# mozilla/mozjpeg

Measured on NVIDIA H100. Metric: megapixels/sec encode (4K RGB q75 4:2:0), higher is better.
Workload: dtype u8 in / int32 DCT / fp32 trellis costs / u8 out

## Files before the change

### mozjpeg_b200/csrc/encoder.cu

```cuda
#include "b200jpeg.h"
#include "internal.h"
#include "kernels.cuh"
#include <cmath>
#include <cstdio>
#include <cstdlib>
#include <cstring>
#include <map>
#include <string>
#include <vector>

namespace b200 {

#define CU(call) do { cudaError_t e_ = (call); if (e_ != cudaSuccess) { set_error("%s failed: %s (%s:%d)", #call, cudaGetErrorString(e_), __FILE__, __LINE__); return B200JPEG_ERR_CUDA; } } while (0)

static const int kZigzag[64] = {
   0,  1,  8, 16,  9,  2,  3, 10, 17, 24, 32, 25, 18, 11,  4,  5,
  12, 19, 26, 33, 40, 48, 41, 34, 27, 20, 13,  6,  7, 14, 21, 28,
  35, 42, 49, 56, 57, 50, 43, 36, 29, 22, 15, 23, 30, 37, 44, 51,
  58, 59, 52, 45, 38, 31, 39, 46, 53, 60, 61, 54, 47, 55, 62, 63};

struct DevBuf {
  void *p = nullptr; size_t cap = 0;
  int reserve(size_t n) {
    if (n <= cap) return B200JPEG_OK;
// ... 611 lines not shown
      }
    }
    auto round = [&](const Geom &gr, const RecLayout &rlr, int bSs, int bSe) -> int {
    if (!pl.progressive) {
      if (fwd_stats) {
        tm.mark("trellis_dc_stats");
        launch_gather_comp_dc(gr, pl.rs, so.dcq, rlr, A.d_hist.as<uint32_t>(), status, n, s);
      } else {
        tm.mark("trellis_stats");
        CU(cudaMemsetAsync(A.d_hist.p, 0, hist_bytes * gr.nc, s));
        launch_gather_comp(gr, pl.rs, A.d_hist.as<uint32_t>(), status, n, s);
      }
      tm.mark("trellis_tables");
      SlotMasks masks; memset(&masks, 0, sizeof masks); masks.period = gr.nc;
      for (int ci = 0; ci < gr.nc; ci++) masks.m[ci] = (1u << gr.c[ci].dc_tbl) | (1u << (4 + gr.c[ci].ac_tbl));
      launch_gen_tables(A.d_hist.as<uint32_t>(), tset, tabset, masks, n * gr.nc, s);
    } else {
      for (int ci = 0; ci < gr.nc; ci++) {
        ScanDesc ts; memset(&ts, 0, sizeof ts);
        ts.ncomps = 1; ts.ci[0] = ci; ts.Ss = bSs; ts.Se = bSe; ts.bim = 1; ts.k_count[0] = 1;
        ts.per_row = gr.c[ci].wib; ts.rows = gr.c[ci].hib; ts.nblocks = (long long)ts.per_row * ts.rows;
        ts.ri = p->restart_in_rows > 0 ? (int)std::min((long long)p->restart_in_rows * ts.per_row, 65535LL) : p->restart_interval;
        tm.mark("trellis_stats");
        CU(cudaMemsetAsync(A.d_hist.p, 0, hist_bytes, s));
        launch_seed_hist(A.d_hist.as<uint32_t>(), 4 + gr.c[ci].ac_tbl, n, s);
        launch_prog_prepare(gr, ts, A.d_blk_aux.as<uint32_t>(), A.d_blk_run.as<uint32_t>(), A.d_blk_mask.as<unsigned long long>(), A.d_tile_bits.as<int>(), A.d_tile_base.as<int>(), n, s);
        launch_gather_prog(gr, ts, A.d_blk_aux.as<uint32_t>(), A.d_blk_run.as<uint32_t>(), A.d_blk_mask.as<unsigned long long>(), A.d_hist.as<uint32_t>(), status, n, s);
        tm.mark("trellis_tables");
        SlotMasks masks; memset(&masks, 0, sizeof masks); masks.period = 1; masks.m[0] = 1u << (4 + gr.c[ci].ac_tbl);
        launch_gen_tables(A.d_hist.as<uint32_t>(), tset + (size_t)ci * HIST_SLOTS, tabset * gr.nc, masks, n, s);
      }
    }
    if (!generic_rounds) {
      tm.mark("trellis_ac");
      if (so.hist) CU(cudaMemsetAsync(A.d_hist.p, 0, hist_bytes, s));
      launch_trellis_ac3(gr, e->d_tc.as<TrellisConsts>(), tset, tabset, A.d_rec.as<DcRec>(), rlr, A.d_srec.p, A.d_splits.as<uint32_t>(), so, n, e->sms, s);
    } else {
      tm.mark("trellis_ac");
      float4 *eo = eobopt ? A.d_eo.as<float4>() : nullptr;
      launch_trellis_ac_band(gr, e->d_tc.as<TrellisConsts>(), tset, tabset, A.d_rec.as<DcRec>(), rlr, bSs, bSe, qimg, eo, n, s);
      if (eobopt) launch_trellis_eob_rows(gr, tset, tabset, A.d_rec.as<DcRec>(), rlr, bSs, bSe, eo, A.d_es.p, n, s);
      if (qopt) launch_qopt_sums(gr, A.d_qsum.as<long long>(), n, s);
    }
    if (p->trellis_quant_dc) {
      tm.mark("trellis_dc");
      if (pl.progressive) launch_trellis_dc(gr, e->d_tc.as<TrellisConsts>(), e->d_tabs_fixed.as<DevHuff>(), 0, A.d_rec.as<DcRec>(), A.d_bt.as<unsigned long long>(), rlr, p->trellis_delta_dc_weight > 0.0f, dc_fast_of(gr), nullptr, 1, n, s);
      else launch_trellis_dc(gr, e->d_tc.as<TrellisConsts>(), tset, tabset, A.d_rec.as<DcRec>(), A.d_bt.as<unsigned long long>(), rlr, p->trellis_delta_dc_weight > 0.0f, dc_fast_of(gr), so.dcq, so.keep_coef, n, s);
    }
    return B200JPEG_OK;
    };
    auto band_Ss = [&](int band) { return (nband == 2 && band == 1) ? p->trellis_freq_split + 1 : 1; };
    auto band_Se = [&](int band) { return (nband == 2 && band == 0) ? p->trellis_freq_split : 63; };
    if (!qopt) {
      for (int loop = 0; loop < p->trellis_num_loops; loop++)
        for (int band = 0; band < nband; band++) { int rc = round(g, rl, band_Ss(band), band_Se(band)); if (rc) return rc; }
    } else {
      const int group = g.nc * (nband == 2 ? 4 : 2);
      int pass_number = 0;
      CU(cudaMemsetAsync(A.d_qsum.p, 0, (size_t)n * 4 * 2 * 64 * 8, s));
      for (int ci = 0; ci < g.nc; ci++) {
        Geom gs = g; gs.nc = 1; gs.c[0] = g.c[ci];
        RecLayout rls = rl; rls.comp_off[0] = rl.comp_off[ci];
        for (int loop = 0; loop < p->trellis_num_loops; loop++)
          for (int band = 0; band < nband; band++) {
            pass_number++;
            if (pass_number % group == 1) CU(cudaMemsetAsync(A.d_qsum.p, 0, (size_t)n * 4 * 2 * 64 * 8, s));
            int rc = round(gs, rls, band_Ss(band), band_Se(band)); if (rc) return rc;
            if ((pass_number + 1) % group == 0) launch_qopt_update(A.d_qsum.as<long long>(), qimg, n, s);
            pass_number++;
          }
      }
      CU(cudaMemcpyAsync(io.qimg, qimg, (size_t)n * 512, cudaMemcpyDeviceToDevice, s));
    }
    if (!fwd_stats) {
      tm.mark("dummy");
      launch_dummy(g, n, s);
    }
  }

  int *best_al = A.d_best_al.as<int>();
// ... 971 lines not shown
```

### mozjpeg_b200/csrc/kernels.cu

```cuda
#include "kernels.cuh"
#include <cuda_fp16.h>
#include <cuda.h>
#include <cstdio>
#include <cstdlib>
#include <type_traits>

namespace b200 {

unsigned long long g_kernel_launches = 0;
#define LAUNCHED() (++g_kernel_launches)

__constant__ uint8_t c_zz[64] = {
   0,  1,  8, 16,  9,  2,  3, 10, 17, 24, 32, 25, 18, 11,  4,  5,
  12, 19, 26, 33, 40, 48, 41, 34, 27, 20, 13,  6,  7, 14, 21, 28,
  35, 42, 49, 56, 57, 50, 43, 36, 29, 22, 15, 23, 30, 37, 44, 51,
  58, 59, 52, 45, 38, 31, 39, 46, 53, 60, 61, 54, 47, 55, 62, 63};
__constant__ uint8_t c_izz[64] = {
   0,  1,  5,  6, 14, 15, 27, 28,  2,  4,  7, 13, 16, 26, 29, 42,
   3,  8, 12, 17, 25, 30, 41, 43,  9, 11, 18, 24, 31, 40, 44, 53,
  10, 19, 23, 32, 39, 45, 52, 54, 20, 22, 33, 38, 46, 51, 55, 60,
  21, 34, 37, 47, 50, 56, 59, 61, 35, 36, 48, 49, 57, 58, 62, 63};
__constant__ unsigned long long c_izz_col[8] = {0x2315140a09030200ull, 0x242216130b080401ull, 0x30252117120c0705ull, 0x312f262018110d06ull, 0x39322e271f19100eull, 0x3a38332d281e1a0full, 0x3e3b37342c291d1bull, 0x3f3d3c36352b2a1cull};
#ifndef FWD_KZ_PACKED
#define FWD_KZ_PACKED 1
// ... 1922 lines not shown
      splits[4 * blockIdx.y] = start[63 - 32]; splits[4 * blockIdx.y + 1] = start[63 - mid_max]; splits[4 * blockIdx.y + 2] = start[63 - 8];
      splits[4 * blockIdx.y + 3] = (uint32_t)nblk;
    }
  }
  __syncthreads();
  if (threadIdx.x < 64) { const unsigned mine = cnt[threadIdx.x]; start[threadIdx.x] += mine ? atomicAdd(&gcur[(size_t)blockIdx.y * 64 + threadIdx.x], mine) : 0u; }
  __syncthreads();
  for (long long b = b0 + threadIdx.x; b < b1; b += blockDim.x) {
    const uint4 q = reinterpret_cast<const uint4 *>(r)[b];
    const int nz = (int)((q.y >> 16) & 0xFF);
    const unsigned pos = atomicAdd(&start[63 - min(nz, 63)], 1u);
    reinterpret_cast<uint4 *>(p)[pos] = make_uint4(q.x, (unsigned)b, q.z, q.w);
  }
}
static void launch_sort2(const Geom &g, const DcRec *rec, const RecLayout &rl, SRec *srec, uint32_t *splits, unsigned *scratch , int mid_max, int n, cudaStream_t s)
{
  long long mb = 0;
  for (int ci = 0; ci < g.nc; ci++) mb = max(mb, (long long)g.c[ci].wib * g.c[ci].hib);
  const size_t words = (size_t)n * g.nc * 64;
  cudaMemsetAsync(scratch, 0, 2 * words * sizeof(unsigned), s);
  dim3 grid((unsigned)((mb + SORT_SLICE - 1) / SORT_SLICE), n * g.nc);
  k_sort_count<<<grid, 256, 0, s>>>(g, rec, rl, scratch); LAUNCHED();
  k_sort_scatter<<<grid, 256, 0, s>>>(g, rec, rl, srec, splits, scratch, scratch + words, mid_max); LAUNCHED();
}

__device__ __forceinline__ float u2f_exact(unsigned v) { return __uint_as_float(0x4B000000u | v) - 8388608.0f; }

#define T3_THREADS 128
#ifndef SYMREC_DIRECT
#define SYMREC_DIRECT 0
#endif
static_assert(!(SYMREC_DIRECT && SYMREC_SPLIT), "the direct-store A/B aid writes whole 128-byte slots");
#ifndef T3_MINB_8
#define T3_MINB_8 8
#endif
#ifndef T3_MINB_15
#define T3_MINB_15 8
#endif
#ifndef T3_PRED_UNROLL
#define T3_PRED_UNROLL 4
#endif
#define T3_PRAGMA_(x) _Pragma(#x)
#define T3_PRAGMA_UNROLL(n) T3_PRAGMA_(unroll n)
template <int MM> struct T3Smem {
  uint2 rec[MM][T3_THREADS];
  unsigned ew[MM][T3_THREADS];
};

template <int KN>
__device__ __forceinline__ void t3_pred_loop(const int t, const uint2 *__restrict__ rec , const unsigned *__restrict__ ew ,
                                             const char *__restrict__ rb, const float before, const float d0, const float d1, const float d2,
                                             float &kb0, int &ks0, float &kb1, int &ks1, float &kb2, int &ks2)
{
T3_PRAGMA_UNROLL(T3_PRED_UNROLL)
  for (int s = 0; s < t; s++) {
    const uint2 r = rec[s * T3_THREADS];
    const int pos4 = (int)(ew[s * T3_THREADS] & 0xFCu);
    const float T = (before + __uint_as_float(r.x)) + __uint_as_float(r.y);
    const char *ra = rb - pos4;
    { const float c = (*reinterpret_cast<const float *>(ra) + d0) + T; if (c < kb0) { kb0 = c; ks0 = s + 1; } }
    if (KN > 1) { const float c = (*reinterpret_cast<const float *>(ra + 256) + d1) + T; if (c < kb1) { kb1 = c; ks1 = s + 1; } }
    if (KN > 2) { const float c = (*reinterpret_cast<const float *>(ra + 512) + d2) + T; if (c < kb2) { kb2 = c; ks2 = s + 1; } }
  }
}
__device__ __forceinline__ float t3_dist(const int cand, const int q, const int x, const float lambda, const float wl)
{
  const float fd = u2f_exact((unsigned)abs(cand * q - x));
  return ((fd * fd) * lambda) * wl;
}

// ... 47 lines not shown
  const size_t rbase = (size_t)img * rl.per_image + rl.comp_off[ci];
  const int use_norm = tc->use_norm;
  const double p1 = tc->p1, p2 = tc->p2; const float lambda_const = tc->lambda_const;
  uint2 *myrec = &L.rec[0][tid]; unsigned *myew = &L.ew[0][tid];
  const char *srate_b = reinterpret_cast<const char *>(srate);
  const float INF = __int_as_float(0x7F800000);

#pragma unroll 1
  for (int chunk = blockIdx.x; chunk < nchunks; chunk += gridDim.x) {
    const long long tix = lo + (long long)chunk * T3_THREADS + tid;
    const bool live = tix < hi;
    SRec sr; sr.norm = 0.f; sr.lin = 0; sr.nzmask = 0;
    if (live) sr = srec[rbase + tix];
    const unsigned lin = sr.lin;
    const int by = lin / c.wib, bx = lin - by * c.wib;
    const size_t blk = ((size_t)img * c.hpad + by) * c.wpad + bx;
    const int16_t *raw16 = c.raw + blk * 64;
    int16_t *o16 = c.coef + blk * 64;
    uint4 rv[8];
#pragma unroll
    for (int v = 0; v < 8; v++) rv[v] = make_uint4(0, 0, 0, 0);
    unsigned dc_q = 0;
    const bool want_dc = !so.sym || so.keep_coef || so.dcq_ac;
    if (live) {
      const uint4 *r4 = reinterpret_cast<const uint4 *>(raw16);
#pragma unroll
      for (int v = 0; v < 8; v++) rv[v] = r4[v];
      if (want_dc) dc_q = (unsigned)(unsigned short)o16[0];
    }
    float lambda;
    {
      const float norm = (float)((double)sr.norm / 63.0);
      if (use_norm) lambda = (float)(p1 / (p2 + (double)norm)); else lambda = lambda_const;
      if (live) rec[rbase + lin].lambda_dc = lambda * swz[0];
    }
    const unsigned mlo = (unsigned)sr.nzmask, mhi = (unsigned)(sr.nzmask >> 32);
    const int m = __popc(mlo) + __popc(mhi);
    const int mmax = __reduce_max_sync(0xffffffffu, m);
    float azd = 0.0f;
    if (mmax != 0) {
      uint2 *push = myrec;
      const float bias = -8421376.0f;
#pragma unroll
      for (int v = 0; v < 8; v++) {
        const unsigned aw[4] = {rv[v].x, rv[v].y, rv[v].z, rv[v].w};
        const float4 w0 = reinterpret_cast<const float4 *>(swz)[2 * v], w1 = reinterpret_cast<const float4 *>(swz)[2 * v + 1];
        const float ww[8] = {w0.x, w0.y, w0.z, w0.w, w1.x, w1.y, w1.z, w1.w};
        const unsigned mw = v < 4 ? mlo : mhi;
#pragma unroll
        for (int jj = 0; jj < 4; jj++) {
          const unsigned u = aw[jj] ^ 0x80008000u;
          const float fx = __fadd_rn(__uint_as_float(__byte_perm(u, 0x4B000000u, 0x7610)), bias);
          const float fy = __fadd_rn(__uint_as_float(__byte_perm(u, 0x4B000000u, 0x7632)), bias);
          const float2 z = make_float2(__fmul_rn(__fmul_rn(__fmul_rn(fx, fx), lambda), ww[2 * jj]),
                                       __fmul_rn(__fmul_rn(__fmul_rn(fy, fy), lambda), ww[2 * jj + 1]));
          const int i = 8 * v + 2 * jj;
          if (i != 0) {
            if (mw & (1u << (i & 31))) { *push = make_uint2(__float_as_uint(azd), __byte_perm(aw[jj], (unsigned)i, 0x1054)); push += T3_THREADS; }
            azd = z.x + azd;
          }
          if (mw & (1u << ((i + 1) & 31))) { *push = make_uint2(__float_as_uint(azd), __byte_perm(aw[jj], (unsigned)(i + 1), 0x3254)); push += T3_THREADS; }
          azd = z.y + azd;
        }
      }
    }
    const float azd63 = azd;
    int last = 0;
// ... 115 lines not shown
#else
        uint4 *dlo = reinterpret_cast<uint4 *>(so.sym + (rbase + lin) * SYMREC_BYTES), *dhi = dlo;
#endif
        for (int v = 0; 4 * v < nw; v += 2) {
          const uint2 a = myrec[(2 * v) * T3_THREADS], b = myrec[(2 * v + 1) * T3_THREADS];
          const uint2 c2 = myrec[(2 * v + 2) * T3_THREADS], d2 = myrec[(2 * v + 3) * T3_THREADS];
          uint4 *dst = v < 4 ? dlo : dhi;
          dst[v] = make_uint4(a.x, a.y, b.x, b.y);
          dst[v + 1] = make_uint4(c2.x, c2.y, d2.x, d2.y);
        }
#endif
        if (so.dcq_ac) so.dcq[rbase + lin] = (int16_t)dc_q;
        if (so.keep_coef || ns > SYMREC_SLOTS) write_block(last0);
      }
    }
  }
  if (so.hist) {
    __syncthreads();
    uint32_t *gh = so.hist + ((size_t)img * HIST_SLOTS + 4 + c.ac_tbl) * HIST_BINS;
    for (int i = tid; i < 162; i += T3_THREADS) {
      const unsigned v = shist[i];
      if (v) atomicAdd(&gh[i < 160 ? (((i / 10) << 4) | (i % 10 + 1)) : i == 160 ? 0 : 0xF0], v);
    }
  }
}

template <int MM>
static void launch_t3(dim3 grid, cudaStream_t s, const Geom &g, const TrellisConsts *tc, const DevHuff *tabs, size_t tabs_set_stride,
                      DcRec *rec, const RecLayout &rl, const SRec *srec, const uint32_t *splits, const SymOut &so)
{
  if (sizeof(T3Smem<MM>) + 8192 > 48 * 1024) cudaFuncSetAttribute(k_trellis_ac3<MM>, cudaFuncAttributeMaxDynamicSharedMemorySize, (int)sizeof(T3Smem<MM>));
  k_trellis_ac3<MM><<<grid, T3_THREADS, sizeof(T3Smem<MM>), s>>>(g, tc, tabs, tabs_set_stride, rec, rl, srec, splits, so); LAUNCHED();
}
void launch_trellis_ac3(const Geom &g, const TrellisConsts *tc, const DevHuff *tabs, size_t tabs_set_stride,
                        DcRec *rec, const RecLayout &rl, void *srec, uint32_t *splits, const SymOut &so, int n, int sms, cudaStream_t s)
{
  launch_sort2(g, rec, rl, static_cast<SRec *>(srec), splits, splits + (size_t)n * g.nc * 4, 15, n, s);
  long long mb = 0;
  for (int ci = 0; ci < g.nc; ci++) mb = max(mb, (long long)g.c[ci].wib * g.c[ci].hib);
  const unsigned full = (unsigned)((mb + T3_THREADS - 1) / T3_THREADS);
  unsigned gx = (unsigned)max(1, min((int)full, (sms * 8 * 3 + n * g.nc - 1) / (n * g.nc)));
  dim3 grid(gx, n * g.nc);
  const SRec *sr = static_cast<const SRec *>(srec);
  launch_t3<64>(dim3(min(gx, 8u), grid.y), s, g, tc, tabs, tabs_set_stride, rec, rl, sr, splits, so);
  launch_t3<32>(dim3(min(gx, 16u), grid.y), s, g, tc, tabs, tabs_set_stride, rec, rl, sr, splits, so);
  launch_t3<15>(grid, s, g, tc, tabs, tabs_set_stride, rec, rl, sr, splits, so);
  launch_t3<8>(grid, s, g, tc, tabs, tabs_set_stride, rec, rl, sr, splits, so);
}

__global__ void __launch_bounds__(256) k_dc_collect(Geom g, RecLayout rl, int16_t *__restrict__ dcq)
{
  const int ci = blockIdx.y % g.nc, img = blockIdx.y / g.nc;
  const CompGeom &c = g.c[ci];
  const long long nblk = (long long)c.wib * c.hib, t = (long long)blockIdx.x * blockDim.x + threadIdx.x;
  if (t >= nblk) return;
  const int row = (int)(t / c.wib), col = (int)(t - (long long)row * c.wib);
  dcq[(size_t)img * rl.per_image + rl.comp_off[ci] + t] = c.coef[(((size_t)img * c.hpad + row) * c.wpad + col) * 64];
}
static void launch_dc_collect(const Geom &g, const RecLayout &rl, int16_t *dcq, int n, cudaStream_t s)
{
  long long mb = 0;
  for (int ci = 0; ci < g.nc; ci++) mb = max(mb, (long long)g.c[ci].wib * g.c[ci].hib);
  dim3 grid((unsigned)((mb + 255) / 256), n * g.nc);
  k_dc_collect<<<grid, 256, 0, s>>>(g, rl, dcq); LAUNCHED();
}

__global__ void __launch_bounds__(64) k_trellis_dc(Geom g, const TrellisConsts *__restrict__ tc,
                                                   const DevHuff *__restrict__ tabs, size_t tabs_set_stride,
                                                   const DcRec *__restrict__ rec, unsigned long long *__restrict__ bt, RecLayout rl)
{
  const int ci = blockIdx.y % g.nc, img = blockIdx.y / g.nc;
  const CompGeom &c = g.c[ci];
  __shared__ uint8_t dcsi[32];
  {
    const DevHuff *dc = reinterpret_cast<const DevHuff *>(reinterpret_cast<const char *>(tabs) + (size_t)blockIdx.y * tabs_set_stride) + c.dc_tbl;
    if (threadIdx.x < 32) dcsi[threadIdx.x] = dc->size[threadIdx.x];
  }
  __syncthreads();
  int imcu = blockIdx.x * blockDim.x + threadIdx.x;
  int n_imcu = (c.hib + c.v - 1) / c.v;
  if (imcu >= n_imcu) return;
  const int q = qset_of(tc, g, img)->q8_zz[c.qt][0];
  int ncand = (2 + 60 / (q >> 3)) | 1; if (ncand > 9) ncand = 9;
  const int half = ncand / 2;
  const int lim = 1 << tc->max_coef_bits;
  int last_dc = 0;
  for (int br = 0; br < c.v; br++) {
    int row = imcu * c.v + br;
    if (row >= c.hib) break;
    size_t rbase = (size_t)img * rl.per_image + rl.comp_off[ci] + (size_t)row * c.wib;
    float acc[9]; int prevc[9];
#pragma unroll
    for (int k = 0; k < 9; k++) { acc[k] = 0.f; prevc[k] = 0; }
    for (int bi = 0; bi < c.wib; bi++) {
      DcRec r = rec[rbase + bi];
      int raw = r.raw_dc, sign = raw >> 31, x = abs(raw);
      int qval = (x + q / 2) / q;
      const bool vert = br > 0 && tc->delta_dc_weight > 0.0f;
      int above_raw = 0, above_fin = 0;
      if (vert) { above_raw = rec[rbase - c.wib + bi].raw_dc; above_fin = c.coef[(((size_t)img * c.hpad + row - 1) * c.wpad + bi) * 64]; }
      float nacc[9]; int cand[9];
      unsigned long long w = 0;
#pragma unroll
      for (int k = 0; k < 9; k++) {
        nacc[k] = 0.f; cand[k] = 0;
        if (k < ncand) {
          int cd = qval - half + k;
          if (cd >= lim) cd = lim - 1;
          if (cd <= -lim) cd = -lim + 1;
          int delta = cd * q - x;
          float dist = (float)(delta * delta) * r.lambda_dc;
          cd *= 1 + 2 * sign;
          cand[k] = cd;
          if (vert) {
            const int d2 = (above_raw - raw) - (above_fin * q - cd * q);
            const float vd = (float)(d2 * d2) * r.lambda_dc;
            dist += tc->delta_dc_weight * (vd - dist);
          }
          if (bi == 0) {
            int bits = nbits_of(abs(cd - last_dc));
            nacc[k] = (float)(bits + dcsi[bits]) + dist;
          } else {
            float best = 0.f; int bl = 0;
#pragma unroll
            for (int l = 0; l < 9; l++) {
              if (l < ncand) {
                int bits = nbits_of(abs(cd - prevc[l]));
                float cost = (float)(bits + dcsi[bits]) + dist + acc[l];
                if (l == 0 || cost < best) { best = cost; bl = l; }
              }
            }
            nacc[k] = best; w |= (unsigned long long)bl << (4 * k);
          }
        }
      }
#pragma unroll
      for (int k = 0; k < 9; k++) { acc[k] = nacc[k]; prevc[k] = cand[k]; }
      w |= (unsigned long long)(qval & 0xFFF) << 36;
      w |= (unsigned long long)(sign & 1) << 48;
      bt[rbase + bi] = w;
    }
    int j = 0; float bj = acc[0];
#pragma unroll
    for (int i = 1; i < 9; i++) if (i < ncand && acc[i] < bj) { bj = acc[i]; j = i; }
    for (int bi = c.wib - 1; bi >= 0; bi--) {
      unsigned long long w = bt[rbase + bi];
      int qval = (int)((w >> 36) & 0xFFF), sg = (int)((w >> 48) & 1);
      int cd = qval - half + j;
      if (cd >= lim) cd = lim - 1;
      if (cd <= -lim) cd = -lim + 1;
      if (sg) cd = -cd;
      c.coef[(((size_t)img * c.hpad + row) * c.wpad + bi) * 64] = (int16_t)cd;
      if (bi == c.wib - 1) last_dc = cd;
      j = (int)((w >> (4 * j)) & 0xF);
    }
  }
}
__global__ void __launch_bounds__(64) k_trellis_dc_warp(Geom g, const TrellisConsts *__restrict__ tc,
                                                        const DevHuff *__restrict__ tabs, size_t tabs_set_stride,
                                                        const DcRec *__restrict__ rec, RecLayout rl, int max_wib)
{
  extern __shared__ unsigned char dsm[];
  const int ci = blockIdx.y % g.nc, img = blockIdx.y / g.nc;
  const CompGeom &c = g.c[ci];
  __shared__ uint8_t dcsi[32];
  {
    const DevHuff *dc = reinterpret_cast<const DevHuff *>(reinterpret_cast<const char *>(tabs) + (size_t)blockIdx.y * tabs_set_stride) + c.dc_tbl;
    if (threadIdx.x < 32) dcsi[threadIdx.x] = dc->size[threadIdx.x];
  }
  __syncthreads();
  const int lane = threadIdx.x & 31, warp = threadIdx.x >> 5;
  const int grp = lane / 9, k = lane - grp * 9;
  const int chain_in_cta = warp * 3 + grp;
  const int chains_per_cta = (blockDim.x >> 5) * 3;
  const int imcu = blockIdx.x * chains_per_cta + chain_in_cta;
  const int n_imcu = (c.hib + c.v - 1) / c.v;
  const bool active = grp < 3 && imcu < n_imcu;
  int16_t *qs = reinterpret_cast<int16_t *>(dsm) + (size_t)chain_in_cta * max_wib;
  uint8_t *bt8 = dsm + (size_t)chains_per_cta * max_wib * 2 + (size_t)chain_in_cta * max_wib * 9;
  tc = qset_of(tc, g, img);
  const int q = tc->q8_zz[c.qt][0];
  int ncand = (2 + 60 / (q >> 3)) | 1; if (ncand > 9) ncand = 9;
  const int half = ncand / 2;
  const int lim = 1 << tc->max_coef_bits;
  const int gbase = grp * 9;
  int last_dc = 0;
  for (int br = 0; br < c.v; br++) {
    int row = imcu * c.v + br;
    bool rowok = active && row < c.hib;
    size_t rbase = (size_t)img * rl.per_image + rl.comp_off[ci] + (size_t)(rowok ? row : 0) * c.wib;
    float acc = 0.f; int prevc = 0;
    DcRec r = rec[rbase];
    for (int bi = 0; bi < c.wib; bi++) {
      DcRec rn = rec[rbase + min(bi + 1, c.wib - 1)];
      int raw = r.raw_dc, sign = raw >> 31, x = abs(raw);
      int qval = (x + q / 2) / q;
      int cd = qval - half + k;
      if (cd >= lim) cd = lim - 1;
      if (cd <= -lim) cd = -lim + 1;
      int delta = cd * q - x;
      float dist = (float)(delta * delta) * r.lambda_dc;
      cd *= 1 + 2 * sign;
      float best; int bl = 0;
      if (bi == 0) {
        int bits = nbits_of(abs(cd - last_dc));
        best = (float)(bits + dcsi[bits]) + dist;
      } else {
        best = 0.f;
#pragma unroll
        for (int l = 0; l < 9; l++) {
          int pc = __shfl_sync(0xffffffffu, prevc, gbase + l);
          float pa = __shfl_sync(0xffffffffu, acc, gbase + l);
          if (l < ncand) {
            int bits = nbits_of(abs(cd - pc));
            float cost = (float)(bits + dcsi[bits]) + dist + pa;
            if (l == 0 || cost < best) { best = cost; bl = l; }
          }
        }
      }
      acc = best; prevc = cd;
      if (rowok && k < ncand) bt8[(size_t)bi * 9 + k] = (uint8_t)bl;
      if (rowok && k == 0) qs[bi] = (int16_t)(sign ? -qval - 1 : qval);
      r = rn;
    }
    int j = 0; float bj = __shfl_sync(0xffffffffu, acc, gbase);
#pragma unroll
    for (int i = 1; i < 9; i++) { float a = __shfl_sync(0xffffffffu, acc, gbase + i); if (i < ncand && a < bj) { bj = a; j = i; } }
    __syncwarp();
    if (rowok && k == 0) {
      for (int bi = c.wib - 1; bi >= 0; bi--) {
        int e = qs[bi]; int sg = e < 0; int qval = sg ? -e - 1 : e;
        int cd = qval - half + j;
        if (cd >= lim) cd = lim - 1;
        if (cd <= -lim) cd = -lim + 1;
        if (sg) cd = -cd;
        c.coef[(((size_t)img * c.hpad + row) * c.wpad + bi) * 64] = (int16_t)cd;
        if (bi == c.wib - 1) last_dc = cd;
        j = bt8[(size_t)bi * 9 + j];
      }
    }
    last_dc = __shfl_sync(0xffffffffu, last_dc, gbase < 27 ? gbase : 0);
    __syncwarp();
  }
}
#ifndef DC2_WARPS
#define DC2_WARPS 2
#endif
#ifndef DC_TABLE
#define DC_TABLE 1
#endif
#define DC_TAB_HALF 512
__device__ __forceinline__ int bfind_u32(unsigned v) { int r; asm("bfind.u32 %0, %1;" : "=r"(r) : "r"(v)); return r; }

template <bool FAST>
__global__ void __launch_bounds__(DC2_WARPS * 32) k_trellis_dc_v2(Geom g, const TrellisConsts *__restrict__ tc,
                                                                 const DevHuff *__restrict__ tabs, size_t tabs_set_stride,
                                                                 const DcRec *__restrict__ rec, RecLayout rl, int max_wib, int16_t *__restrict__ dcq, int write_coef)
{
  extern __shared__ __align__(16) unsigned char dsm[];
  __shared__ float T[36];
  __shared__ float Tt[(FAST && DC_TABLE) ? 2 * DC_TAB_HALF + 8 : 1];
  __shared__ int4 stage[DC2_WARPS][3][32];
  const int ci = blockIdx.y % g.nc, img = blockIdx.y / g.nc;
  const CompGeom &c = g.c[ci];
  {
    const DevHuff *dc = reinterpret_cast<const DevHuff *>(reinterpret_cast<const char *>(tabs) + (size_t)blockIdx.y * tabs_set_stride) + c.dc_tbl;
    if (threadIdx.x < 33) T[threadIdx.x] = (float)((int)threadIdx.x + (int)dc->size[threadIdx.x & 255]);
  }
  __syncthreads();
  if (FAST && DC_TABLE) {
    for (int i = threadIdx.x; i < 2 * DC_TAB_HALF + 8; i += DC2_WARPS * 32) Tt[i] = T[1 + bfind_u32((unsigned)abs(i - DC_TAB_HALF))];
    __syncthreads();
  }
  const int lane = threadIdx.x & 31, warp = threadIdx.x >> 5;
  const int grp = lane / 9, k = lane - grp * 9;
  const int gsel = grp < 3 ? grp : 0;
  const int gbase = gsel * 9;
  const int n_imcu = (c.hib + c.v - 1) / c.v;
  const int imcu0 = (blockIdx.x * DC2_WARPS + warp) * 3;
  const int wib = c.wib;
  uint8_t *btw = dsm + (size_t)warp * 3 * max_wib * 5;
  uint8_t *bt = btw + (size_t)gsel * max_wib * 5;
  tc = qset_of(tc, g, img);
  const int q = tc->q8_zz[c.qt][0];
  int ncand = (2 + 60 / (q >> 3)) | 1; if (ncand > 9) ncand = 9;
  const int half = ncand / 2;
  const int lim = 1 << tc->max_coef_bits;
  const float INF = __int_as_float(0x7f800000);
  const size_t comp_rec = (size_t)img * rl.per_image + rl.comp_off[ci];
  const int qhalf = q / 2;
  const unsigned qmul = tc->dc_mul[c.qt]; const int qshift = tc->dc_shift[c.qt];
  int last_dc = 0;
  for (int br = 0; br < c.v; br++) {
    int rowg[3]; bool okg[3];
#pragma unroll
    for (int gg = 0; gg < 3; gg++) { int r = (imcu0 + gg) * c.v + br; okg[gg] = (imcu0 + gg) < n_imcu && r < c.hib; rowg[gg] = okg[gg] ? r : 0; }
    const bool rowok = grp < 3 && okg[gsel];
    DcRec nxt[3];
#pragma unroll
    for (int gg = 0; gg < 3; gg++) nxt[gg] = rec[comp_rec + (size_t)rowg[gg] * wib + min(lane, wib - 1)];
    float acc = 0.f;
    int pbase = last_dc, psgn = 1, pstep = 0;
    uint8_t *btp = bt + (k >> 1);
    for (int bi0 = 0; bi0 < wib; bi0 += 32) {
      __syncwarp();
#pragma unroll
      for (int gg = 0; gg < 3; gg++) {
        const int raw = nxt[gg].raw_dc, x = abs(raw);
        const int qval = (int)(((unsigned long long)(unsigned)(x + qhalf) * qmul) >> qshift);
        stage[warp][gg][lane] = make_int4(x, qval - half, 1 + 2 * (raw >> 31), __float_as_int(nxt[gg].lambda_dc));
      }
      __syncwarp();
      if (bi0 + 32 < wib) {
#pragma unroll
        for (int gg = 0; gg < 3; gg++) nxt[gg] = rec[comp_rec + (size_t)rowg[gg] * wib + min(bi0 + 32 + lane, wib - 1)];
      }
      const int nstep = min(32, wib - bi0);
      const int4 *sp = &stage[warp][gsel][0];
#pragma unroll 1
      for (int st = 0; st < nstep; st++) {
        const int4 r = sp[st];
        const int x = r.x, base = r.y, sgn = r.z;
        int cd = base + k;
        if (!FAST) { if (cd >= lim) cd = lim - 1; if (cd <= -lim) cd = -lim + 1; }
        const int delta = cd * q - x;
        const float dist = (float)(delta * delta) * __int_as_float(r.w);
        cd *= sgn;
        float rd[9];
        if (FAST) {
          const int D0 = cd - psgn * pbase, dstep = -psgn * pstep;
          const int E0 = dstep < 0 ? -D0 : D0;
          if (DC_TABLE && __all_sync(0xffffffffu, pstep != 0 && (unsigned)(E0 + DC_TAB_HALF) < (unsigned)(2 * DC_TAB_HALF))) {
            const float *tp = Tt + (E0 + DC_TAB_HALF);
#pragma unroll
            for (int l = 0; l < 9; l++) rd[l] = tp[l] + dist;
          } else {
#pragma unroll
            for (int l = 0; l < 9; l++) rd[l] = T[1 + bfind_u32((unsigned)abs(D0 + dstep * l))] + dist;
          }
        } else {
#pragma unroll
          for (int l = 0; l < 9; l++) {
            int v = pbase + pstep * l;
// ... 33 lines not shown
#pragma unroll 4
      for (int bi = wib - 1; bi >= 0; bi--) {
        uint8_t *bb = bt + (size_t)bi * 5;
        const int byte = bb[j >> 1];
        const int jn = (j & 1) ? (byte >> 4) : (byte & 15);
        bb[4] = (uint8_t)((bb[4] & 15) | (j << 4));
        j = jn;
      }
    }
    __syncwarp();
#pragma unroll
    for (int gg = 0; gg < 3; gg++) {
      const uint8_t *btg = btw + (size_t)gg * max_wib * 5;
      int lastv = 0;
      for (int bi = lane; bi < wib && okg[gg]; bi += 32) {
        DcRec r = rec[comp_rec + (size_t)rowg[gg] * wib + bi];
        int raw = r.raw_dc, sign = raw >> 31, x = abs(raw);
        int cdv = (int)(((unsigned long long)(unsigned)(x + qhalf) * qmul) >> qshift) - half + (btg[(size_t)bi * 5 + 4] >> 4);
        if (cdv >= lim) cdv = lim - 1;
        if (cdv <= -lim) cdv = -lim + 1;
        if (sign) cdv = -cdv;
        if (write_coef) c.coef[(((size_t)img * c.hpad + rowg[gg]) * c.wpad + bi) * 64] = (int16_t)cdv;
        if (dcq) dcq[comp_rec + (size_t)rowg[gg] * wib + bi] = (int16_t)cdv;
        if (bi == wib - 1) lastv = cdv;
      }
      lastv = __shfl_sync(0xffffffffu, lastv, (wib - 1) & 31);
      if (grp == gg) last_dc = lastv;
    }
    __syncwarp();
  }
}

void launch_trellis_dc(const Geom &g, const TrellisConsts *tc, const DevHuff *tabs, size_t tabs_set_stride,
                       const DcRec *rec, unsigned long long *bt, const RecLayout &rl, int vertical, int dc_fast, int16_t *dcq, int write_coef, int n, cudaStream_t s)
{
  int n_imcu = 0, max_wib = 0;
  for (int ci = 0; ci < g.nc; ci++) { n_imcu = max(n_imcu, (g.c[ci].hib + g.c[ci].v - 1) / g.c[ci].v); max_wib = max(max_wib, g.c[ci].wib); }
  if (vertical) {
    dim3 grid((n_imcu + 63) / 64, n * g.nc);
    k_trellis_dc<<<grid, 64, 0, s>>>(g, tc, tabs, tabs_set_stride, rec, bt, rl);
    LAUNCHED();
    if (dcq) launch_dc_collect(g, rl, dcq, n, s);
    return;
  }
  static const bool use_v1 = getenv("B200JPEG_DC_V1") != nullptr;
  size_t smem2 = (size_t)DC2_WARPS * 3 * max_wib * 5;
  if (!use_v1 && smem2 <= 200 * 1024) {
    if (smem2 > 40 * 1024) { cudaFuncSetAttribute(k_trellis_dc_v2<true>, cudaFuncAttributeMaxDynamicSharedMemorySize, 200 * 1024); cudaFuncSetAttribute(k_trellis_dc_v2<false>, cudaFuncAttributeMaxDynamicSharedMemorySize, 200 * 1024); }
    dim3 grid((n_imcu + DC2_WARPS * 3 - 1) / (DC2_WARPS * 3), n * g.nc);
    if (dc_fast) k_trellis_dc_v2<true><<<grid, DC2_WARPS * 32, smem2, s>>>(g, tc, tabs, tabs_set_stride, rec, rl, max_wib, dcq, write_coef || !dcq);
    else k_trellis_dc_v2<false><<<grid, DC2_WARPS * 32, smem2, s>>>(g, tc, tabs, tabs_set_stride, rec, rl, max_wib, dcq, write_coef || !dcq);
    LAUNCHED();
    return;
  }
  int warps = 2;
  size_t smem = (size_t)warps * 3 * max_wib * 11;
  if (smem > 200 * 1024) { warps = 1; smem = (size_t)3 * max_wib * 11; }
  if (smem <= 200 * 1024) {
    if (smem > 48 * 1024) cudaFuncSetAttribute(k_trellis_dc_warp, cudaFuncAttributeMaxDynamicSharedMemorySize, 200 * 1024);
    dim3 grid((n_imcu + warps * 3 - 1) / (warps * 3), n * g.nc);
    k_trellis_dc_warp<<<grid, warps * 32, smem, s>>>(g, tc, tabs, tabs_set_stride, rec, rl, max_wib);
  } else {
    dim3 grid((n_imcu + 63) / 64, n * g.nc);
    k_trellis_dc<<<grid, 64, 0, s>>>(g, tc, tabs, tabs_set_stride, rec, bt, rl);
  }
  LAUNCHED();
  if (dcq) launch_dc_collect(g, rl, dcq, n, s);
}

struct ScanTables {
  uint16_t code[HIST_SLOTS][256];
  uint8_t size[HIST_SLOTS][256];
};
__device__ __forceinline__ void load_scan_tables(ScanTables &st, const DevHuff *tabs, size_t stride, int img, const Geom &g, const ScanDesc &sd, bool want_codes)
{
  const DevHuff *t = reinterpret_cast<const DevHuff *>(reinterpret_cast<const char *>(tabs) + (size_t)img * stride);
  for (int i = 0; i < sd.ncomps; i++) {
    const CompGeom &c = g.c[sd.ci[i]];
    int slots[2] = {c.dc_tbl, 4 + c.ac_tbl};
    for (int z = 0; z < 2; z++) {
      int sl = slots[z];
      for (int k = threadIdx.x; k < 256; k += blockDim.x) { st.size[sl][k] = t[sl].size[k]; if (want_codes) st.code[sl][k] = t[sl].code[k]; }
    }
  }
}

struct CountSink {
  const uint8_t *dsz, *asz; unsigned bits; int bad;
  __device__ void dc(int nb, int) { int s = dsz[nb]; if (!s) bad = 1; bits += s + nb; }
  __device__ void ac(int sym, int nb, int) { int s = asz[sym]; if (!s) bad = 1; bits += s + nb; }
};

__device__ __forceinline__ unsigned cta_sum_256(unsigned v, unsigned *ws )
{
  for (int o = 16; o; o >>= 1) v += __shfl_xor_sync(0xffffffffu, v, o);
  if ((threadIdx.x & 31) == 0) ws[threadIdx.x >> 5] = v;
  __syncthreads();
// ... 943 lines not shown
```

### mozjpeg_b200/csrc/kernels.cuh

```cuda
#pragma once
#include <cstdint>
#include <cuda_runtime.h>

namespace b200 {

struct CompGeom {
  int wib, hib;
  int wpad, hpad;
  int h, v;
  int hx, vx;
  int qt;
  int dc_tbl, ac_tbl;
  int rows_avail;
  long long blocks_per_image;
  int16_t *coef, *raw;
};
struct RestartSpec { int interval, in_rows; };
struct Geom {
  int W, H, nc, hmax, vmax;
  int mcus_per_row, mcu_rows;
  int in_comps;
  int max_coef_bits;
  int cs_mode;
  int px_first, px_swap;
// ... 46 lines not shown
  uint8_t  size[256];
};
static_assert(sizeof(DevHuff) == 17 + 256 + 1 + 12 + 2 + 512 + 256, "DevHuff layout");

struct DcRec { float lambda_dc; int16_t raw_dc; uint8_t nz; uint8_t pad; unsigned long long nzmask; };
static_assert(sizeof(DcRec) == 16, "DcRec layout");
struct RecLayout { long long per_image; long long comp_off[4]; long long sym_hi; };
struct SlotMasks { uint32_t m[4]; int period; };

#define SYMREC_BYTES 128
#define SYMREC_SLOTS 31
#ifndef SYMREC_SPLIT
#define SYMREC_SPLIT 1
#endif
struct SymOut { uint8_t *sym; int16_t *dcq; uint32_t *hist; int keep_coef; int dcq_ac; };

#define HIST_BINS 257
#define HIST_SLOTS 8

void launch_prep_planes(const Geom &g, const uint8_t *src, int smoothing_factor, const PlanesOut &out, int n, cudaStream_t s);
struct YuvOut { uint8_t *p[3]; size_t pitch[3], stride[3]; int pw[3], ph[3]; };
void launch_encode_yuv(const Geom &g, const uint8_t *src, const YuvOut &out, int n, cudaStream_t s);
void launch_import_coefs(const Geom &g, int n, cudaStream_t s);
struct FwdStats { uint32_t *hist; int16_t *dcq; uint32_t *status; };
bool forward_tiled(const Geom &g, int dct_method);
void launch_forward(const Geom &g, const uint8_t *src, const QuantTables *qt, int qfast, int dct_method , int dering, DcRec *rec, const RecLayout &rl, int keep_raw,
                    const FwdStats &fs, int n, cudaStream_t s);
void launch_dummy(const Geom &g, int n, cudaStream_t s);
void launch_gather_comp(const Geom &g, const RestartSpec &rs, uint32_t *hist, uint32_t *status, int n, cudaStream_t s);
void launch_gather_comp_dc(const Geom &g, const RestartSpec &rs, const int16_t *dcq, const RecLayout &rl, uint32_t *hist, uint32_t *status, int n, cudaStream_t s);
void launch_gather_seq(const Geom &g, const ScanDesc &sd, const DcRec *nz_rec, const uint8_t *sym, const int16_t *dcq, const RecLayout &rl, uint32_t *hist, uint32_t *status, int n, cudaStream_t s);
void launch_seed_hist(uint32_t *hist, int slot, int n, cudaStream_t s);
void launch_gen_tables(const uint32_t *hist, DevHuff *tabs, size_t tabs_set_stride, const SlotMasks &masks, int nsets, cudaStream_t s);
void launch_trellis_ac3(const Geom &g, const TrellisConsts *tc, const DevHuff *tabs, size_t tabs_set_stride,
                        DcRec *rec, const RecLayout &rl, void *srec, uint32_t *splits, const SymOut &so, int n, int sms, cudaStream_t s);
void launch_trellis_ac_band(const Geom &g, const TrellisConsts *tc, const DevHuff *tabs, size_t tabs_set_stride,
                            DcRec *rec, const RecLayout &rl, int Ss, int Se, const uint16_t *qimg, float4 *eo, int n, cudaStream_t s);
void launch_trellis_eob_rows(const Geom &g, const DevHuff *tabs, size_t tabs_set_stride, DcRec *rec, const RecLayout &rl, int Ss, int Se,
                             const float4 *eo, void *scratch, int n, cudaStream_t s);
void launch_qopt_sums(const Geom &g, long long *qsum, int n, cudaStream_t s);
void launch_qopt_update(long long *qsum, uint16_t *qimg, int n, cudaStream_t s);
void launch_trellis_dc(const Geom &g, const TrellisConsts *tc, const DevHuff *tabs, size_t tabs_set_stride,
                       const DcRec *rec, unsigned long long *bt, const RecLayout &rl, int vertical, int dc_fast, int16_t *dcq, int write_coef, int n, cudaStream_t s);
void launch_gather_seq_dc(const Geom &g, const ScanDesc &sd, const int16_t *dcq, const RecLayout &rl, uint32_t *hist, uint32_t *status, int n, cudaStream_t s);
void launch_prog_prepare(const Geom &g, const ScanDesc &sd, uint32_t *aux, uint32_t *run_e, unsigned long long *pm, int *tile_last, int *tile_first, int n, cudaStream_t s);
void launch_gather_prog(const Geom &g, const ScanDesc &sd, const uint32_t *aux, const uint32_t *run_e, const unsigned long long *pm, uint32_t *hist, uint32_t *status, int n, cudaStream_t s);
void launch_block_bits(const Geom &g, const ScanDesc &sd, const DcRec *nz_rec, const uint8_t *sym, const int16_t *dcq, const RecLayout &rl, const DevHuff *tabs, size_t tabs_image_stride, int progressive,
                       uint32_t *blk_bits, uint32_t *tile_bits, const uint32_t *blk_aux, const uint32_t *run_e, const unsigned long long *pm, uint32_t *status, int n, cudaStream_t s);
void launch_scan_layout(const ScanDesc &sd, const uint32_t *blk_bits, const uint32_t *tile_bits, unsigned long long *tile_base,
                        uint32_t *seg_corr, long long seg_stride, unsigned long long *total_bits, size_t capacity_bits,
                        uint32_t *status, int n, cudaStream_t s);
void launch_zero_stream(uint32_t *bitbuf, size_t bitbuf_image_stride_words, const unsigned long long *total_bits, int n, cudaStream_t s);
void launch_encode(const Geom &g, const ScanDesc &sd, const DcRec *nz_rec, const uint8_t *sym, const int16_t *dcq, const RecLayout &rl, const DevHuff *tabs, size_t tabs_image_stride, int progressive,
                   const uint32_t *blk_bits, const uint32_t *tile_bits, const unsigned long long *tile_base, const uint32_t *seg_corr, long long seg_stride,
                   const uint32_t *blk_aux, const uint32_t *run_e, const unsigned long long *pm,
                   uint32_t *bitbuf, size_t bitbuf_image_stride_words, uint32_t *mark, size_t mark_stride_words, const uint32_t *status, int n, cudaStream_t s);
size_t stuff_tiles(size_t bitbuf_image_stride_words);
size_t stuff_lookback_bytes(size_t bitbuf_image_stride_words, int n);
void launch_stuff(const uint32_t *bitbuf, size_t bitbuf_image_stride_words, const unsigned long long *total_bits, void *lookback,
                  uint8_t *out, size_t out_image_stride, size_t out_capacity, const unsigned long long *out_start, unsigned long long *out_next,
                  uint32_t *scan_size, uint32_t *status, const uint32_t *mark, size_t mark_stride_words, int n, cudaStream_t s);

void launch_lossless_diff(const Geom &g, const ScanDesc &sd, int precision, const uint8_t *src, uint16_t *diff, uint32_t *hist, int n, cudaStream_t s);
void launch_lossless_bits(const Geom &g, const ScanDesc &sd, const uint16_t *diff, const DevHuff *tabs, size_t tabs_image_stride,
                          uint32_t *blk_bits, uint32_t *tile_bits, uint32_t *status, int n, cudaStream_t s);
void launch_lossless_encode(const Geom &g, const ScanDesc &sd, const uint16_t *diff, const DevHuff *tabs, size_t tabs_image_stride,
                            const uint32_t *blk_bits, const unsigned long long *tile_base, const uint32_t *seg_corr, long long seg_stride,
                            uint32_t *bitbuf, size_t bitbuf_image_stride_words, uint32_t *mark, size_t mark_stride_words, const uint32_t *status, int n, cudaStream_t s);

struct AlSearch { ScanDesc sd[24]; int first, per_al, nband, al_max, nscans_total; };
void launch_select_al(const Geom &g, const AlSearch &as, const DevHuff *tabs_scan, const uint32_t *scan_size, int n, int *best_al, cudaStream_t s);

extern unsigned long long g_kernel_launches;

}
```

Before: 60090.

## Recompute DC trellis lambda from norm instead of storing it in AC trellis

The AC trellis kernel no longer writes a per-block lambda_dc into the record array. The DC trellis kernels instead recompute lambda from the stored norm and the DC weight when running the non-generic path, which removes a scattered global store from the hot AC kernel. The sort launch is split out of the AC launcher into its own call, and the AC kernel's minimum blocks per SM drops from 8 to 6, which allows more registers per thread. The trade is extra division and double-precision arithmetic in the DC kernels, and a risk of register or occupancy changes in the AC kernel.

```diff
diff --git a/mozjpeg_b200/csrc/encoder.cu b/mozjpeg_b200/csrc/encoder.cu
--- a/mozjpeg_b200/csrc/encoder.cu
+++ b/mozjpeg_b200/csrc/encoder.cu
@@ -667,6 +667,8 @@
       }
     }
     if (!generic_rounds) {
+      tm.mark("trellis_sort");
+      launch_trellis_sort(gr, A.d_rec.as<DcRec>(), rlr, A.d_srec.p, A.d_splits.as<uint32_t>(), n, s);
       tm.mark("trellis_ac");
       if (so.hist) CU(cudaMemsetAsync(A.d_hist.p, 0, hist_bytes, s));
       launch_trellis_ac3(gr, e->d_tc.as<TrellisConsts>(), tset, tabset, A.d_rec.as<DcRec>(), rlr, A.d_srec.p, A.d_splits.as<uint32_t>(), so, n, e->sms, s);
@@ -679,8 +681,9 @@
     }
     if (p->trellis_quant_dc) {
       tm.mark("trellis_dc");
-      if (pl.progressive) launch_trellis_dc(gr, e->d_tc.as<TrellisConsts>(), e->d_tabs_fixed.as<DevHuff>(), 0, A.d_rec.as<DcRec>(), A.d_bt.as<unsigned long long>(), rlr, p->trellis_delta_dc_weight > 0.0f, dc_fast_of(gr), nullptr, 1, n, s);
-      else launch_trellis_dc(gr, e->d_tc.as<TrellisConsts>(), tset, tabset, A.d_rec.as<DcRec>(), A.d_bt.as<unsigned long long>(), rlr, p->trellis_delta_dc_weight > 0.0f, dc_fast_of(gr), so.dcq, so.keep_coef, n, s);
+      const int lambda_from_norm = generic_rounds ? 0 : 1;
+      if (pl.progressive) launch_trellis_dc(gr, e->d_tc.as<TrellisConsts>(), e->d_tabs_fixed.as<DevHuff>(), 0, A.d_rec.as<DcRec>(), A.d_bt.as<unsigned long long>(), rlr, p->trellis_delta_dc_weight > 0.0f, dc_fast_of(gr), nullptr, 1, lambda_from_norm, n, s);
+      else launch_trellis_dc(gr, e->d_tc.as<TrellisConsts>(), tset, tabset, A.d_rec.as<DcRec>(), A.d_bt.as<unsigned long long>(), rlr, p->trellis_delta_dc_weight > 0.0f, dc_fast_of(gr), so.dcq, so.keep_coef, lambda_from_norm, n, s);
     }
     return B200JPEG_OK;
     };
diff --git a/mozjpeg_b200/csrc/kernels.cu b/mozjpeg_b200/csrc/kernels.cu
--- a/mozjpeg_b200/csrc/kernels.cu
+++ b/mozjpeg_b200/csrc/kernels.cu
@@ -1978,10 +1978,10 @@
 #endif
 static_assert(!(SYMREC_DIRECT && SYMREC_SPLIT), "the direct-store A/B aid writes whole 128-byte slots");
 #ifndef T3_MINB_8
-#define T3_MINB_8 8
+#define T3_MINB_8 6
 #endif
 #ifndef T3_MINB_15
-#define T3_MINB_15 8
+#define T3_MINB_15 6
 #endif
 #ifndef T3_PRED_UNROLL
 #define T3_PRED_UNROLL 4
@@ -2095,7 +2095,6 @@
     {
       const float norm = (float)((double)sr.norm / 63.0);
       if (use_norm) lambda = (float)(p1 / (p2 + (double)norm)); else lambda = lambda_const;
-      if (live) rec[rbase + lin].lambda_dc = lambda * swz[0];
     }
     const unsigned mlo = (unsigned)sr.nzmask, mhi = (unsigned)(sr.nzmask >> 32);
     const int m = __popc(mlo) + __popc(mhi);
@@ -2277,10 +2276,13 @@
   if (sizeof(T3Smem<MM>) + 8192 > 48 * 1024) cudaFuncSetAttribute(k_trellis_ac3<MM>, cudaFuncAttributeMaxDynamicSharedMemorySize, (int)sizeof(T3Smem<MM>));
   k_trellis_ac3<MM><<<grid, T3_THREADS, sizeof(T3Smem<MM>), s>>>(g, tc, tabs, tabs_set_stride, rec, rl, srec, splits, so); LAUNCHED();
 }
+void launch_trellis_sort(const Geom &g, const DcRec *rec, const RecLayout &rl, void *srec, uint32_t *splits, int n, cudaStream_t s)
+{
+  launch_sort2(g, rec, rl, static_cast<SRec *>(srec), splits, splits + (size_t)n * g.nc * 4, 15, n, s);
+}
 void launch_trellis_ac3(const Geom &g, const TrellisConsts *tc, const DevHuff *tabs, size_t tabs_set_stride,
-                        DcRec *rec, const RecLayout &rl, void *srec, uint32_t *splits, const SymOut &so, int n, int sms, cudaStream_t s)
-{
-  launch_sort2(g, rec, rl, static_cast<SRec *>(srec), splits, splits + (size_t)n * g.nc * 4, 15, n, s);
+                        DcRec *rec, const RecLayout &rl, const void *srec, const uint32_t *splits, const SymOut &so, int n, int sms, cudaStream_t s)
+{
   long long mb = 0;
   for (int ci = 0; ci < g.nc; ci++) mb = max(mb, (long long)g.c[ci].wib * g.c[ci].hib);
   const unsigned full = (unsigned)((mb + T3_THREADS - 1) / T3_THREADS);
@@ -2310,9 +2312,17 @@
   k_dc_collect<<<grid, 256, 0, s>>>(g, rl, dcq); LAUNCHED();
 }
 
+__device__ __forceinline__ float dc_lambda(const float f, const int from_norm, const TrellisConsts *__restrict__ tc, const float w0)
+{
+  if (!from_norm) return f;
+  const float norm = __fdiv_rn(f, 63.0f);
+  const float lambda = tc->use_norm ? (float)(tc->p1 / (tc->p2 + (double)norm)) : tc->lambda_const;
+  return lambda * w0;
+}
+
 __global__ void __launch_bounds__(64) k_trellis_dc(Geom g, const TrellisConsts *__restrict__ tc,
                                                    const DevHuff *__restrict__ tabs, size_t tabs_set_stride,
-                                                   const DcRec *__restrict__ rec, unsigned long long *__restrict__ bt, RecLayout rl)
+                                                   const DcRec *__restrict__ rec, unsigned long long *__restrict__ bt, RecLayout rl, int lambda_from_norm)
 {
   const int ci = blockIdx.y % g.nc, img = blockIdx.y / g.nc;
   const CompGeom &c = g.c[ci];
@@ -2326,6 +2336,7 @@
   int n_imcu = (c.hib + c.v - 1) / c.v;
   if (imcu >= n_imcu) return;
   const int q = qset_of(tc, g, img)->q8_zz[c.qt][0];
+  const float w0 = qset_of(tc, g, img)->w_zz[c.qt][0];
   int ncand = (2 + 60 / (q >> 3)) | 1; if (ncand > 9) ncand = 9;
   const int half = ncand / 2;
   const int lim = 1 << tc->max_coef_bits;
@@ -2341,6 +2352,7 @@
       DcRec r = rec[rbase + bi];
       int raw = r.raw_dc, sign = raw >> 31, x = abs(raw);
       int qval = (x + q / 2) / q;
+      const float lambda_dc = dc_lambda(r.lambda_dc, lambda_from_norm, tc, w0);
       const bool vert = br > 0 && tc->delta_dc_weight > 0.0f;
       int above_raw = 0, above_fin = 0;
       if (vert) { above_raw = rec[rbase - c.wib + bi].raw_dc; above_fin = c.coef[(((size_t)img * c.hpad + row - 1) * c.wpad + bi) * 64]; }
@@ -2354,12 +2366,12 @@
           if (cd >= lim) cd = lim - 1;
           if (cd <= -lim) cd = -lim + 1;
           int delta = cd * q - x;
-          float dist = (float)(delta * delta) * r.lambda_dc;
+          float dist = (float)(delta * delta) * lambda_dc;
           cd *= 1 + 2 * sign;
           cand[k] = cd;
           if (vert) {
             const int d2 = (above_raw - raw) - (above_fin * q - cd * q);
-            const float vd = (float)(d2 * d2) * r.lambda_dc;
+            const float vd = (float)(d2 * d2) * lambda_dc;
             dist += tc->delta_dc_weight * (vd - dist);
           }
           if (bi == 0) {
@@ -2403,7 +2415,7 @@
 }
 __global__ void __launch_bounds__(64) k_trellis_dc_warp(Geom g, const TrellisConsts *__restrict__ tc,
                                                         const DevHuff *__restrict__ tabs, size_t tabs_set_stride,
-                                                        const DcRec *__restrict__ rec, RecLayout rl, int max_wib)
+                                                        const DcRec *__restrict__ rec, RecLayout rl, int max_wib, int lambda_from_norm)
 {
   extern __shared__ unsigned char dsm[];
   const int ci = blockIdx.y % g.nc, img = blockIdx.y / g.nc;
@@ -2425,6 +2437,7 @@
   uint8_t *bt8 = dsm + (size_t)chains_per_cta * max_wib * 2 + (size_t)chain_in_cta * max_wib * 9;
   tc = qset_of(tc, g, img);
   const int q = tc->q8_zz[c.qt][0];
+  const float w0 = tc->w_zz[c.qt][0];
   int ncand = (2 + 60 / (q >> 3)) | 1; if (ncand > 9) ncand = 9;
   const int half = ncand / 2;
   const int lim = 1 << tc->max_coef_bits;
@@ -2444,7 +2457,7 @@
       if (cd >= lim) cd = lim - 1;
       if (cd <= -lim) cd = -lim + 1;
       int delta = cd * q - x;
-      float dist = (float)(delta * delta) * r.lambda_dc;
+      float dist = (float)(delta * delta) * dc_lambda(r.lambda_dc, lambda_from_norm, tc, w0);
       cd *= 1 + 2 * sign;
       float best; int bl = 0;
       if (bi == 0) {
@@ -2500,7 +2513,8 @@
 template <bool FAST>
 __global__ void __launch_bounds__(DC2_WARPS * 32) k_trellis_dc_v2(Geom g, const TrellisConsts *__restrict__ tc,
                                                                  const DevHuff *__restrict__ tabs, size_t tabs_set_stride,
-                                                                 const DcRec *__restrict__ rec, RecLayout rl, int max_wib, int16_t *__restrict__ dcq, int write_coef)
+                                                                 const DcRec *__restrict__ rec, RecLayout rl, int max_wib, int16_t *__restrict__ dcq, int write_coef,
+                                                                 int lambda_from_norm)
 {
   extern __shared__ __align__(16) unsigned char dsm[];
   __shared__ float T[36];
@@ -2528,6 +2542,7 @@
   uint8_t *bt = btw + (size_t)gsel * max_wib * 5;
   tc = qset_of(tc, g, img);
   const int q = tc->q8_zz[c.qt][0];
+  const float w0 = tc->w_zz[c.qt][0];
   int ncand = (2 + 60 / (q >> 3)) | 1; if (ncand > 9) ncand = 9;
   const int half = ncand / 2;
   const int lim = 1 << tc->max_coef_bits;
@@ -2553,7 +2568,7 @@
       for (int gg = 0; gg < 3; gg++) {
         const int raw = nxt[gg].raw_dc, x = abs(raw);
         const int qval = (int)(((unsigned long long)(unsigned)(x + qhalf) * qmul) >> qshift);
-        stage[warp][gg][lane] = make_int4(x, qval - half, 1 + 2 * (raw >> 31), __float_as_int(nxt[gg].lambda_dc));
+        stage[warp][gg][lane] = make_int4(x, qval - half, 1 + 2 * (raw >> 31), __float_as_int(dc_lambda(nxt[gg].lambda_dc, lambda_from_norm, tc, w0)));
       }
       __syncwarp();
       if (bi0 + 32 < wib) {
@@ -2653,13 +2668,14 @@
 }
 
 void launch_trellis_dc(const Geom &g, const TrellisConsts *tc, const DevHuff *tabs, size_t tabs_set_stride,
-                       const DcRec *rec, unsigned long long *bt, const RecLayout &rl, int vertical, int dc_fast, int16_t *dcq, int write_coef, int n, cudaStream_t s)
+                       const DcRec *rec, unsigned long long *bt, const RecLayout &rl, int vertical, int dc_fast, int16_t *dcq, int write_coef,
+                       int lambda_from_norm, int n, cudaStream_t s)
 {
   int n_imcu = 0, max_wib = 0;
   for (int ci = 0; ci < g.nc; ci++) { n_imcu = max(n_imcu, (g.c[ci].hib + g.c[ci].v - 1) / g.c[ci].v); max_wib = max(max_wib, g.c[ci].wib); }
   if (vertical) {
     dim3 grid((n_imcu + 63) / 64, n * g.nc);
-    k_trellis_dc<<<grid, 64, 0, s>>>(g, tc, tabs, tabs_set_stride, rec, bt, rl);
+    k_trellis_dc<<<grid, 64, 0, s>>>(g, tc, tabs, tabs_set_stride, rec, bt, rl, lambda_from_norm);
     LAUNCHED();
     if (dcq) launch_dc_collect(g, rl, dcq, n, s);
     return;
@@ -2669,8 +2685,8 @@
   if (!use_v1 && smem2 <= 200 * 1024) {
     if (smem2 > 40 * 1024) { cudaFuncSetAttribute(k_trellis_dc_v2<true>, cudaFuncAttributeMaxDynamicSharedMemorySize, 200 * 1024); cudaFuncSetAttribute(k_trellis_dc_v2<false>, cudaFuncAttributeMaxDynamicSharedMemorySize, 200 * 1024); }
     dim3 grid((n_imcu + DC2_WARPS * 3 - 1) / (DC2_WARPS * 3), n * g.nc);
-    if (dc_fast) k_trellis_dc_v2<true><<<grid, DC2_WARPS * 32, smem2, s>>>(g, tc, tabs, tabs_set_stride, rec, rl, max_wib, dcq, write_coef || !dcq);
-    else k_trellis_dc_v2<false><<<grid, DC2_WARPS * 32, smem2, s>>>(g, tc, tabs, tabs_set_stride, rec, rl, max_wib, dcq, write_coef || !dcq);
+    if (dc_fast) k_trellis_dc_v2<true><<<grid, DC2_WARPS * 32, smem2, s>>>(g, tc, tabs, tabs_set_stride, rec, rl, max_wib, dcq, write_coef || !dcq, lambda_from_norm);
+    else k_trellis_dc_v2<false><<<grid, DC2_WARPS * 32, smem2, s>>>(g, tc, tabs, tabs_set_stride, rec, rl, max_wib, dcq, write_coef || !dcq, lambda_from_norm);
     LAUNCHED();
     return;
   }
@@ -2680,10 +2696,10 @@
   if (smem <= 200 * 1024) {
     if (smem > 48 * 1024) cudaFuncSetAttribute(k_trellis_dc_warp, cudaFuncAttributeMaxDynamicSharedMemorySize, 200 * 1024);
     dim3 grid((n_imcu + warps * 3 - 1) / (warps * 3), n * g.nc);
-    k_trellis_dc_warp<<<grid, warps * 32, smem, s>>>(g, tc, tabs, tabs_set_stride, rec, rl, max_wib);
+    k_trellis_dc_warp<<<grid, warps * 32, smem, s>>>(g, tc, tabs, tabs_set_stride, rec, rl, max_wib, lambda_from_norm);
   } else {
     dim3 grid((n_imcu + 63) / 64, n * g.nc);
-    k_trellis_dc<<<grid, 64, 0, s>>>(g, tc, tabs, tabs_set_stride, rec, bt, rl);
+    k_trellis_dc<<<grid, 64, 0, s>>>(g, tc, tabs, tabs_set_stride, rec, bt, rl, lambda_from_norm);
   }
   LAUNCHED();
   if (dcq) launch_dc_collect(g, rl, dcq, n, s);
diff --git a/mozjpeg_b200/csrc/kernels.cuh b/mozjpeg_b200/csrc/kernels.cuh
--- a/mozjpeg_b200/csrc/kernels.cuh
+++ b/mozjpeg_b200/csrc/kernels.cuh
@@ -102,8 +102,9 @@
 void launch_gather_seq(const Geom &g, const ScanDesc &sd, const DcRec *nz_rec, const uint8_t *sym, const int16_t *dcq, const RecLayout &rl, uint32_t *hist, uint32_t *status, int n, cudaStream_t s);
 void launch_seed_hist(uint32_t *hist, int slot, int n, cudaStream_t s);
 void launch_gen_tables(const uint32_t *hist, DevHuff *tabs, size_t tabs_set_stride, const SlotMasks &masks, int nsets, cudaStream_t s);
+void launch_trellis_sort(const Geom &g, const DcRec *rec, const RecLayout &rl, void *srec, uint32_t *splits, int n, cudaStream_t s);
 void launch_trellis_ac3(const Geom &g, const TrellisConsts *tc, const DevHuff *tabs, size_t tabs_set_stride,
-                        DcRec *rec, const RecLayout &rl, void *srec, uint32_t *splits, const SymOut &so, int n, int sms, cudaStream_t s);
+                        DcRec *rec, const RecLayout &rl, const void *srec, const uint32_t *splits, const SymOut &so, int n, int sms, cudaStream_t s);
 void launch_trellis_ac_band(const Geom &g, const TrellisConsts *tc, const DevHuff *tabs, size_t tabs_set_stride,
                             DcRec *rec, const RecLayout &rl, int Ss, int Se, const uint16_t *qimg, float4 *eo, int n, cudaStream_t s);
 void launch_trellis_eob_rows(const Geom &g, const DevHuff *tabs, size_t tabs_set_stride, DcRec *rec, const RecLayout &rl, int Ss, int Se,
@@ -111,7 +112,8 @@
 void launch_qopt_sums(const Geom &g, long long *qsum, int n, cudaStream_t s);
 void launch_qopt_update(long long *qsum, uint16_t *qimg, int n, cudaStream_t s);
 void launch_trellis_dc(const Geom &g, const TrellisConsts *tc, const DevHuff *tabs, size_t tabs_set_stride,
-                       const DcRec *rec, unsigned long long *bt, const RecLayout &rl, int vertical, int dc_fast, int16_t *dcq, int write_coef, int n, cudaStream_t s);
+                       const DcRec *rec, unsigned long long *bt, const RecLayout &rl, int vertical, int dc_fast, int16_t *dcq, int write_coef,
+                       int lambda_from_norm, int n, cudaStream_t s);
 void launch_gather_seq_dc(const Geom &g, const ScanDesc &sd, const int16_t *dcq, const RecLayout &rl, uint32_t *hist, uint32_t *status, int n, cudaStream_t s);
 void launch_prog_prepare(const Geom &g, const ScanDesc &sd, uint32_t *aux, uint32_t *run_e, unsigned long long *pm, int *tile_last, int *tile_first, int n, cudaStream_t s);
 void launch_gather_prog(const Geom &g, const ScanDesc &sd, const uint32_t *aux, const uint32_t *run_e, const unsigned long long *pm, uint32_t *hist, uint32_t *status, int n, cudaStream_t s);
```

New measurement: 62520, median of 6. 4.0% higher.
